# zju3dv/Diffuman4D

Measured on NVIDIA H100. Metric: unet_window_denoise_steps_per_sec, higher is better.
Workload: dtype bf16

## Files before the change

diffuman4d_b200/csrc/attention_wgmma.cu:

```cuda
#include <math.h>

#include "kernels.h"
#include "wgmma.cuh"

namespace d4d {

namespace {

constexpr int BLOCK_Q = 128;
constexpr int BLOCK_KV = 64;
constexpr int ATT_THREADS = 288;
constexpr int QBOX_BYTES = BLOCK_Q * 64 * 2;
constexpr int KVBOX_BYTES = BLOCK_KV * 64 * 2;

template <int NB>
struct AttCfg {
  static constexpr int D = 64 * NB;
  static constexpr int STAGES = NB == 3 ? 3 : 4;
  static constexpr int Q_BYTES = QBOX_BYTES * NB;
  static constexpr int STAGE_BYTES = 2 * KVBOX_BYTES * NB;
  static constexpr int SMEM_BYTES = 1024 + Q_BYTES + STAGES * STAGE_BYTES + 256;
  static constexpr int MIN_BLOCKS = NB == 1 ? 2 : 1;
};

struct AttKernelArgs {
  int seq_q, seq_kv, heads, n_kv_tiles;
  float scale_log2;
  bf16* out;
  int ld_out;
};

__device__ __forceinline__ float ex2_approx(float x) {
  float y;
  asm("ex2.approx.ftz.f32 %0, %1;" : "=f"(y) : "f"(x));
  return y;
}

template <int NB>
__global__ void __launch_bounds__(ATT_THREADS, AttCfg<NB>::MIN_BLOCKS)
attn_wgmma_kernel(const __grid_constant__ CUtensorMap tmap_q, const __grid_constant__ CUtensorMap tmap_k,
                  const __grid_constant__ CUtensorMap tmap_v, const AttKernelArgs a) {
  using C = AttCfg<NB>;
  extern __shared__ uint8_t smem_raw[];
  uint8_t* smem = reinterpret_cast<uint8_t*>((reinterpret_cast<uintptr_t>(smem_raw) + 1023) & ~uintptr_t(1023));
  uint8_t* sQ = smem;
  uint8_t* ring = smem + C::Q_BYTES;
  uint64_t* kv_full = reinterpret_cast<uint64_t*>(ring + C::STAGES * C::STAGE_BYTES);
  uint64_t* kv_empty = kv_full + C::STAGES;
  uint64_t* q_full = kv_empty + C::STAGES;

  const int warp = __shfl_sync(0xffffffffu, threadIdx.x >> 5, 0);
  const int lane = threadIdx.x & 31;
  const int q_tile = blockIdx.x;
  const int bh = blockIdx.y;
  const int b = bh / a.heads;
  const int hd = bh - b * a.heads;
  const int q_row0 = b * a.seq_q;
  const int kv_row0 = b * a.seq_kv;
  const int col0 = hd * C::D;
  const int n_tiles = a.n_kv_tiles;

  if (threadIdx.x == 0) {
    for (int i = 0; i < C::STAGES; ++i) {
      mbar_init(&kv_full[i], 1);
      mbar_init(&kv_empty[i], 2);
    }
    mbar_init(q_full, 1);
    fence_mbar_init();
  }
  __syncthreads();
  pdl_wait();
  pdl_launch_dependents();

  if (warp == 8) {
    if (lane == 0) {
      tma_prefetch_desc(&tmap_q);
      tma_prefetch_desc(&tmap_k);
      tma_prefetch_desc(&tmap_v);
      mbar_expect_tx(q_full, C::Q_BYTES);
#pragma unroll
      for (int nb = 0; nb < NB; ++nb)
        tma_load_2d(sQ + nb * QBOX_BYTES, &tmap_q, q_full, col0 + nb * 64, q_row0 + q_tile * BLOCK_Q);
      int stage = 0;
      uint32_t phase = 0;
      for (int j = 0; j < n_tiles; ++j) {
        mbar_wait(&kv_empty[stage], phase ^ 1);
        uint8_t* dst = ring + stage * C::STAGE_BYTES;
        mbar_expect_tx(&kv_full[stage], C::STAGE_BYTES);
#pragma unroll
        for (int nb = 0; nb < NB; ++nb) {
          tma_load_2d(dst + nb * KVBOX_BYTES, &tmap_k, &kv_full[stage], col0 + nb * 64, kv_row0 + j * BLOCK_KV);
          tma_load_2d(dst + (NB + nb) * KVBOX_BYTES, &tmap_v, &kv_full[stage], col0 + nb * 64, kv_row0 + j * BLOCK_KV);
        }
        if (++stage == C::STAGES) { stage = 0; phase ^= 1; }
      }
    }
    return;
  }

  const int wg = warp >> 2;
  const bool wg_leader = (threadIdx.x & 127) == 0;
  const int c_base = 2 * (lane & 3);
  const uint32_t q_addr = smem_u32(sQ) + wg * 64 * 128;
  const uint32_t ring_u32 = smem_u32(ring);

  float o[NB][32];
#pragma unroll
  for (int nb = 0; nb < NB; ++nb)
#pragma unroll
    for (int i = 0; i < 32; ++i) o[nb][i] = 0.f;
  float m_run[2] = {-INFINITY, -INFINITY};
  float l_run[2] = {0.f, 0.f};
  mbar_wait(q_full, 0);

  int stage = 0;
  uint32_t phase = 0;
  for (int j = 0; j < n_tiles; ++j) {
    mbar_wait(&kv_full[stage], phase);
    const uint32_t kv = ring_u32 + stage * C::STAGE_BYTES;
    float s[32];
    wgmma_fence();
#pragma unroll
    for (int nb = 0; nb < NB; ++nb) {
      const uint64_t qd = make_wgmma_desc(q_addr + nb * QBOX_BYTES, 16, 1024);
      const uint64_t kd = make_wgmma_desc(kv + nb * KVBOX_BYTES, 16, 1024);
#pragma unroll
      for (int k = 0; k < 4; ++k) wgmma_ss_n64(s, qd + 2 * k, kd + 2 * k, (nb | k) != 0 ? 1 : 0);
    }
    wgmma_commit();
    wgmma_wait<0>();
    wgmma_fence_regs(s);

    const int valid = a.seq_kv - j * BLOCK_KV;
    if (valid < BLOCK_KV) {
#pragma unroll
      for (int i = 0; i < 32; ++i)
        if (8 * (i >> 2) + c_base + (i & 1) >= valid) s[i] = -INFINITY;
    }
    float corr[2];
#pragma unroll
    for (int h = 0; h < 2; ++h) {
      float mx = -INFINITY;
#pragma unroll
      for (int jj = 0; jj < 8; ++jj) mx = fmaxf(mx, fmaxf(s[4 * jj + 2 * h], s[4 * jj + 2 * h + 1]));
      mx = fmaxf(mx, __shfl_xor_sync(0xffffffffu, mx, 1));
      mx = fmaxf(mx, __shfl_xor_sync(0xffffffffu, mx, 2));
      const float m_new = fmaxf(m_run[h], mx * a.scale_log2);
      corr[h] = ex2_approx(m_run[h] - m_new);
      m_run[h] = m_new;
      float sum = 0.f;
#pragma unroll
      for (int jj = 0; jj < 8; ++jj) {
#pragma unroll
        for (int e = 0; e < 2; ++e) {
          const float p = ex2_approx(fmaf(s[4 * jj + 2 * h + e], a.scale_log2, -m_new));
          s[4 * jj + 2 * h + e] = p;
          sum += p;
        }
      }
      l_run[h] = l_run[h] * corr[h] + sum;
    }
#pragma unroll
    for (int nb = 0; nb < NB; ++nb)
#pragma unroll
      for (int i = 0; i < 32; ++i) o[nb][i] *= corr[(i >> 1) & 1];

    uint32_t pf[4][4];
#pragma unroll
    for (int kk = 0; kk < 4; ++kk) {
      pf[kk][0] = pack_bf16x2(s[8 * kk + 0], s[8 * kk + 1]);
      pf[kk][1] = pack_bf16x2(s[8 * kk + 2], s[8 * kk + 3]);
      pf[kk][2] = pack_bf16x2(s[8 * kk + 4], s[8 * kk + 5]);
      pf[kk][3] = pack_bf16x2(s[8 * kk + 6], s[8 * kk + 7]);
    }
    wgmma_fence();
#pragma unroll
    for (int nb = 0; nb < NB; ++nb) {
      const uint64_t vd = make_wgmma_desc(kv + (NB + nb) * KVBOX_BYTES, KVBOX_BYTES, 1024);
#pragma unroll
      for (int kk = 0; kk < 4; ++kk) wgmma_rs_n64_bmn(o[nb], pf[kk], vd + (2048 >> 4) * kk);
    }
    wgmma_commit();
    wgmma_wait<0>();
#pragma unroll
    for (int nb = 0; nb < NB; ++nb) wgmma_fence_regs(o[nb]);
    if (wg_leader) mbar_arrive(&kv_empty[stage]);
    if (++stage == C::STAGES) { stage = 0; phase ^= 1; }
  }

  const int r_base = q_tile * BLOCK_Q + wg * 64 + (warp & 3) * 16 + (lane >> 2);
#pragma unroll
  for (int h = 0; h < 2; ++h) {
    float l = l_run[h];
    l += __shfl_xor_sync(0xffffffffu, l, 1);
    l += __shfl_xor_sync(0xffffffffu, l, 2);
    const float inv_l = 1.f / l;
    const int qrow = r_base + 8 * h;
    if (qrow >= a.seq_q) continue;
    bf16* orow = a.out + static_cast<size_t>(q_row0 + qrow) * a.ld_out + col0;
#pragma unroll
    for (int nb = 0; nb < NB; ++nb)
#pragma unroll
      for (int jj = 0; jj < 8; ++jj)
        *reinterpret_cast<uint32_t*>(orow + nb * 64 + 8 * jj + c_base) =
            pack_bf16x2(o[nb][4 * jj + 2 * h] * inv_l, o[nb][4 * jj + 2 * h + 1] * inv_l);
  }
}

template <int NB>
int launch_attn(const AttnLaunch& L, cudaStream_t stream) {
  using C = AttCfg<NB>;
  static PerDeviceOnce attr_once;
  if (int rc = ensure_dyn_smem(attn_wgmma_kernel<NB>, C::SMEM_BYTES, attr_once)) return rc;
  AttKernelArgs a;
  a.seq_q = L.d.seq;
  a.seq_kv = L.d.seq_kv > 0 ? L.d.seq_kv : L.d.seq;
  a.heads = L.d.heads;
  a.n_kv_tiles = (a.seq_kv + BLOCK_KV - 1) / BLOCK_KV;
  a.scale_log2 = L.d.scale * 1.4426950408889634f;
  a.out = L.d.out;
  a.ld_out = L.d.ld_out;
  dim3 grid(L.grid_x, L.grid_y);
  D4D_CUDA_OK(launch_pdl(attn_wgmma_kernel<NB>, grid, dim3(ATT_THREADS), C::SMEM_BYTES, stream, L.tmap_q, L.tmap_k, L.tmap_v, a));
  D4D_CUDA_OK(cudaGetLastError());
  return 0;
}

}

int attn_prepare(const AttnDesc& d, AttnLaunch* L) {
  D4D_REQUIRE(d.head_dim == 64 || d.head_dim == 128 || d.head_dim == 192,
              "attention head_dim (after padding) must be 64, 128 or 192");
  D4D_REQUIRE(d.batch > 0 && d.seq > 0 && d.heads > 0 && d.seq_kv >= 0, "empty attention problem");
  D4D_REQUIRE(d.ld_qkv % 8 == 0 && d.ld_out % 8 == 0 && d.ld_kv % 8 == 0, "leading dimensions must be multiples of 8");
  D4D_REQUIRE(d.scale > 0.f, "softmax scale must be positive");
  L->d = d;
  L->variant = d.head_dim / 64;
  const int seq_kv = d.seq_kv > 0 ? d.seq_kv : d.seq;
  const int ld_kv = d.ld_kv > 0 ? d.ld_kv : d.ld_qkv;
  const uint64_t q_tokens = static_cast<uint64_t>(d.batch) * d.seq;
  const uint64_t kv_tokens = static_cast<uint64_t>(d.batch) * seq_kv;
  const uint64_t width = static_cast<uint64_t>(d.heads) * d.head_dim;
  if (int rc = make_tmap_2d(&L->tmap_q, d.q, q_tokens, width, d.ld_qkv, 64, BLOCK_Q, 128)) return rc;
  if (int rc = make_tmap_2d(&L->tmap_k, d.k, kv_tokens, width, ld_kv, 64, BLOCK_KV, 128)) return rc;
  if (int rc = make_tmap_2d(&L->tmap_v, d.v, kv_tokens, width, ld_kv, 64, BLOCK_KV, 128)) return rc;
  L->grid_x = (d.seq + BLOCK_Q - 1) / BLOCK_Q;
  L->grid_y = d.batch * d.heads;
  D4D_REQUIRE(L->grid_y <= 65535, "batch*heads exceeds grid.y limit");
  return 0;
}

int attn_run(const AttnLaunch& L, cudaStream_t stream) {
  switch (L.variant) {
    case 1: return launch_attn<1>(L, stream);
    case 2: return launch_attn<2>(L, stream);
    case 3: return launch_attn<3>(L, stream);
  }
  set_error("attention: unsupported head_dim variant");
  return 1;
}

double attn_flops(const AttnDesc& d) {
  const double skv = d.seq_kv > 0 ? d.seq_kv : d.seq;
  return 4.0 * d.batch * d.heads * static_cast<double>(d.seq) * skv * d.head_dim;
}

}
```

diffuman4d_b200/csrc/common.cuh:

```cuda
#pragma once
#include <cuda.h>
#include <cuda_bf16.h>
#include <cuda_runtime.h>
#include <stdint.h>
#include <string>

namespace d4d {

typedef __nv_bfloat16 bf16;

void set_error(const std::string& msg);
#define D4D_CUDA_OK(expr)                                                                        \
  do {                                                                                           \
    cudaError_t _e = (expr);                                                                     \
    if (_e != cudaSuccess) {                                                                     \
      d4d::set_error(std::string(#expr) + " failed: " + cudaGetErrorString(_e) + " @" + __FILE__ + \
                     ":" + std::to_string(__LINE__));                                            \
      return 2;                                                                                  \
    }                                                                                            \
  } while (0)
#define D4D_REQUIRE(cond, msg)                                                                   \
  do {                                                                                           \
    if (!(cond)) {                                                                               \
      d4d::set_error(std::string("invalid argument: ") + msg + " (" #cond ") @" + __FILE__ + ":" + \
                     std::to_string(__LINE__));                                                  \
      return 1;                                                                                  \
    }                                                                                            \
  } while (0)

int make_tmap_2d(CUtensorMap* out, const void* base, uint64_t rows, uint64_t cols, uint64_t ld,
                 uint32_t box_cols, uint32_t box_rows, int swizzle_bytes);
int make_tmap_nhwc(CUtensorMap* out, const void* base, uint64_t n, uint64_t h, uint64_t w, uint64_t c,
                   uint32_t box_c, uint32_t box_w, uint32_t box_h, uint32_t box_n, int swizzle_bytes, int stride = 1);

#ifdef __CUDACC__
__device__ __forceinline__ uint32_t smem_u32(const void* p) {
  return static_cast<uint32_t>(__cvta_generic_to_shared(p));
}
__device__ __forceinline__ bool elect_one() {
  uint32_t pred = 0;
  asm volatile(
      "{\n\t.reg .b32 rx;\n\t.reg .pred px;\n\t"
      "elect.sync rx|px, 0xffffffff;\n\t"
      "selp.b32 %0, 1, 0, px;\n\t}\n"
      : "=r"(pred));
  return pred != 0;
}

__device__ __forceinline__ void mbar_init(uint64_t* bar, uint32_t count) {
  asm volatile("mbarrier.init.shared::cta.b64 [%0], %1;" ::"r"(smem_u32(bar)), "r"(count) : "memory");
}
__device__ __forceinline__ void fence_mbar_init() {
  asm volatile("fence.mbarrier_init.release.cluster;" ::: "memory");
}
__device__ __forceinline__ void mbar_expect_tx(uint64_t* bar, uint32_t bytes) {
  asm volatile("mbarrier.arrive.expect_tx.shared::cta.b64 _, [%0], %1;" ::"r"(smem_u32(bar)), "r"(bytes)
               : "memory");
}
__device__ __forceinline__ void mbar_arrive(uint64_t* bar) {
  asm volatile("mbarrier.arrive.shared::cta.b64 _, [%0];" ::"r"(smem_u32(bar)) : "memory");
}
__device__ __forceinline__ bool mbar_try_wait(uint64_t* bar, uint32_t parity) {
  uint32_t ok;
  asm volatile(
      "{\n\t.reg .pred p;\n\t"
      "mbarrier.try_wait.parity.shared::cta.b64 p, [%1], %2;\n\t"
      "selp.b32 %0, 1, 0, p;\n\t}\n"
      : "=r"(ok)
      : "r"(smem_u32(bar)), "r"(parity)
      : "memory");
  return ok != 0;
}
#ifndef D4D_SPIN_LIMIT
#define D4D_SPIN_LIMIT (1u << 26)
#endif
__device__ __forceinline__ void mbar_wait(uint64_t* bar, uint32_t parity) {
  uint32_t spins = 0;
  while (!mbar_try_wait(bar, parity)) {
    if (++spins > D4D_SPIN_LIMIT) {
      printf("d4d: mbarrier timeout block=(%d,%d) thread=%d bar=%u parity=%u\n", blockIdx.x, blockIdx.y,
             threadIdx.x, smem_u32(bar), parity);
      __trap();
    }
  }
}

__device__ __forceinline__ void fence_proxy_async_smem() {
  asm volatile("fence.proxy.async.shared::cta;" ::: "memory");
}
__device__ __forceinline__ void named_barrier_sync(int id, int threads) {
  asm volatile("bar.sync %0, %1;" ::"r"(id), "r"(threads) : "memory");
}
__device__ __forceinline__ void st_shared_u32(uint32_t addr, uint32_t v) {
  asm volatile("st.shared.b32 [%0], %1;" ::"r"(addr), "r"(v) : "memory");
}
__device__ __forceinline__ uint32_t ld_shared_u32(uint32_t addr) {
  uint32_t v;
  asm volatile("ld.shared.b32 %0, [%1];" : "=r"(v) : "r"(addr) : "memory");
  return v;
}
__device__ __forceinline__ void pdl_wait() { asm volatile("griddepcontrol.wait;" ::: "memory"); }
__device__ __forceinline__ void pdl_launch_dependents() { asm volatile("griddepcontrol.launch_dependents;" ::: "memory"); }
template <int R> __device__ __forceinline__ void setmaxnreg_dec() { asm volatile("setmaxnreg.dec.sync.aligned.u32 %0;" ::"n"(R)); }
template <int R> __device__ __forceinline__ void setmaxnreg_inc() { asm volatile("setmaxnreg.inc.sync.aligned.u32 %0;" ::"n"(R)); }

__device__ __forceinline__ void tma_prefetch_desc(const CUtensorMap* t) {
  asm volatile("prefetch.tensormap [%0];" ::"l"(reinterpret_cast<uint64_t>(t)) : "memory");
}
__device__ __forceinline__ void tma_load_2d(void* dst, const CUtensorMap* t, uint64_t* bar, int c0, int c1) {
  asm volatile(
      "cp.async.bulk.tensor.2d.shared::cluster.global.tile.mbarrier::complete_tx::bytes [%0], [%1, {%3, %4}], [%2];"
      ::"r"(smem_u32(dst)), "l"(reinterpret_cast<uint64_t>(t)), "r"(smem_u32(bar)), "r"(c0), "r"(c1)
      : "memory");
}
__device__ __forceinline__ void tma_load_4d(void* dst, const CUtensorMap* t, uint64_t* bar, int c0, int c1, int c2,
                                            int c3) {
  asm volatile(
      "cp.async.bulk.tensor.4d.shared::cluster.global.tile.mbarrier::complete_tx::bytes [%0], [%1, {%3, %4, %5, %6}], [%2];"
      ::"r"(smem_u32(dst)), "l"(reinterpret_cast<uint64_t>(t)), "r"(smem_u32(bar)), "r"(c0), "r"(c1), "r"(c2),
      "r"(c3)
      : "memory");
}

__device__ __forceinline__ void tma_store_2d(const CUtensorMap* t, const void* src, int c0, int c1) {
  asm volatile("cp.async.bulk.tensor.2d.global.shared::cta.bulk_group [%0, {%2, %3}], [%1];"
               ::"l"(reinterpret_cast<uint64_t>(t)), "r"(smem_u32(src)), "r"(c0), "r"(c1) : "memory");
}
__device__ __forceinline__ void bulk_commit_group() { asm volatile("cp.async.bulk.commit_group;" ::: "memory"); }
template <int N> __device__ __forceinline__ void bulk_wait_group_read() {
  asm volatile("cp.async.bulk.wait_group.read %0;" ::"n"(N) : "memory");
}
template <int N> __device__ __forceinline__ void bulk_wait_group() {
  asm volatile("cp.async.bulk.wait_group %0;" ::"n"(N) : "memory");
}

__device__ __forceinline__ uint32_t pack_bf16x2(float lo, float hi) {
  __nv_bfloat162 v = __floats2bfloat162_rn(lo, hi);
  return *reinterpret_cast<uint32_t*>(&v);
}
__device__ __forceinline__ float2 unpack_bf16x2(uint32_t u) {
  __nv_bfloat162 v = *reinterpret_cast<__nv_bfloat162*>(&u);
  return __bfloat1622float2(v);
}
__device__ __forceinline__ float silu_f(float x) { return __fdividef(x, 1.0f + __expf(-x)); }
__device__ __forceinline__ float gelu_erf_f(float g) {
  const float u = fabsf(g);
  float q = fmaf(-4.8811754095e-04f, u, 7.1988063864e-03f);
  q = fmaf(q, u, -5.2146803588e-02f);
  q = fmaf(q, u, -4.5959571004e-01f);
  q = fmaf(q, u, -1.1510006189e+00f);
  float e;
  asm("ex2.approx.ftz.f32 %0, %1;" : "=f"(e) : "f"(q * u));
  return fmaf(-0.5f * u, e, fmaxf(g, 0.f));
}
#endif

}
```

Baseline: 13.33.

## Skip flash-attention output rescale unless running max grows past slack threshold

The online softmax now only updates the running max and rescales the output accumulators when a tile's max exceeds the current running max by more than a slack (8 in log2 units), checked warp-uniformly with __any_sync. Otherwise it keeps the stale max, which avoids the per-tile multiply over all output registers and the correction exp. Separately, the mbarrier waits switch to a lean variant with no printf or diagnostics on timeout, to cut code size and register pressure in the hot loop. The risk is that exponents up to 2^8 can feed into the bf16 P packing and fp32 accumulators before a rescale happens, which is numerically tolerable but changes rounding slightly.

New measurement: 13.68, median of 6. 1.03x the previous value.

```diff
diff --git a/diffuman4d_b200/csrc/attention_wgmma.cu b/diffuman4d_b200/csrc/attention_wgmma.cu
--- a/diffuman4d_b200/csrc/attention_wgmma.cu
+++ b/diffuman4d_b200/csrc/attention_wgmma.cu
@@ -22,6 +22,11 @@
   static constexpr int SMEM_BYTES = 1024 + Q_BYTES + STAGES * STAGE_BYTES + 256;
   static constexpr int MIN_BLOCKS = NB == 1 ? 2 : 1;
 };
+
+#ifndef D4D_ATTN_RESCALE_SLACK
+#define D4D_ATTN_RESCALE_SLACK 8.f
+#endif
+constexpr float RESCALE_SLACK = D4D_ATTN_RESCALE_SLACK;
 
 struct AttKernelArgs {
   int seq_q, seq_kv, heads, n_kv_tiles;
@@ -84,7 +89,7 @@
       int stage = 0;
       uint32_t phase = 0;
       for (int j = 0; j < n_tiles; ++j) {
-        mbar_wait(&kv_empty[stage], phase ^ 1);
+        mbar_wait_nocall(&kv_empty[stage], phase ^ 1);
         uint8_t* dst = ring + stage * C::STAGE_BYTES;
         mbar_expect_tx(&kv_full[stage], C::STAGE_BYTES);
 #pragma unroll
@@ -111,12 +116,12 @@
     for (int i = 0; i < 32; ++i) o[nb][i] = 0.f;
   float m_run[2] = {-INFINITY, -INFINITY};
   float l_run[2] = {0.f, 0.f};
-  mbar_wait(q_full, 0);
+  mbar_wait_nocall(q_full, 0);
 
   int stage = 0;
   uint32_t phase = 0;
   for (int j = 0; j < n_tiles; ++j) {
-    mbar_wait(&kv_full[stage], phase);
+    mbar_wait_nocall(&kv_full[stage], phase);
     const uint32_t kv = ring_u32 + stage * C::STAGE_BYTES;
     float s[32];
     wgmma_fence();
@@ -137,7 +142,8 @@
       for (int i = 0; i < 32; ++i)
         if (8 * (i >> 2) + c_base + (i & 1) >= valid) s[i] = -INFINITY;
     }
-    float corr[2];
+    float m_tile[2];
+    bool moves = false;
 #pragma unroll
     for (int h = 0; h < 2; ++h) {
       float mx = -INFINITY;
@@ -145,25 +151,37 @@
       for (int jj = 0; jj < 8; ++jj) mx = fmaxf(mx, fmaxf(s[4 * jj + 2 * h], s[4 * jj + 2 * h + 1]));
       mx = fmaxf(mx, __shfl_xor_sync(0xffffffffu, mx, 1));
       mx = fmaxf(mx, __shfl_xor_sync(0xffffffffu, mx, 2));
-      const float m_new = fmaxf(m_run[h], mx * a.scale_log2);
-      corr[h] = ex2_approx(m_run[h] - m_new);
-      m_run[h] = m_new;
+      m_tile[h] = mx * a.scale_log2;
+      moves |= m_tile[h] > m_run[h] + RESCALE_SLACK;
+    }
+    float corr[2] = {1.f, 1.f};
+    if (__any_sync(0xffffffffu, moves)) {
+#pragma unroll
+      for (int h = 0; h < 2; ++h) {
+        if (m_tile[h] > m_run[h] + RESCALE_SLACK) {
+          corr[h] = ex2_approx(m_run[h] - m_tile[h]);
+          m_run[h] = m_tile[h];
+        }
+      }
+#pragma unroll
+      for (int nb = 0; nb < NB; ++nb)
+#pragma unroll
+        for (int i = 0; i < 32; ++i) o[nb][i] *= corr[(i >> 1) & 1];
+    }
+#pragma unroll
+    for (int h = 0; h < 2; ++h) {
       float sum = 0.f;
 #pragma unroll
       for (int jj = 0; jj < 8; ++jj) {
 #pragma unroll
         for (int e = 0; e < 2; ++e) {
-          const float p = ex2_approx(fmaf(s[4 * jj + 2 * h + e], a.scale_log2, -m_new));
+          const float p = ex2_approx(fmaf(s[4 * jj + 2 * h + e], a.scale_log2, -m_run[h]));
           s[4 * jj + 2 * h + e] = p;
           sum += p;
         }
       }
       l_run[h] = l_run[h] * corr[h] + sum;
     }
-#pragma unroll
-    for (int nb = 0; nb < NB; ++nb)
-#pragma unroll
-      for (int i = 0; i < 32; ++i) o[nb][i] *= corr[(i >> 1) & 1];
 
     uint32_t pf[4][4];
 #pragma unroll
diff --git a/diffuman4d_b200/csrc/common.cuh b/diffuman4d_b200/csrc/common.cuh
--- a/diffuman4d_b200/csrc/common.cuh
+++ b/diffuman4d_b200/csrc/common.cuh
@@ -84,6 +84,12 @@
     }
   }
 }
+__device__ __forceinline__ void mbar_wait_nocall(uint64_t* bar, uint32_t parity) {
+  uint32_t spins = 0;
+  while (!mbar_try_wait(bar, parity)) {
+    if (++spins > D4D_SPIN_LIMIT) __trap();
+  }
+}
 
 __device__ __forceinline__ void fence_proxy_async_smem() {
   asm volatile("fence.proxy.async.shared::cta;" ::: "memory");
```
